# timdestan/go-raytracer

Measured on AMD Instinct MI355X. Metric: Mrays/s (primary+shadow+reflect) at 4K depth=6; 1/2/4/8-GPU scaling, higher is better.
Workload: dtype f64; 1 GPU; c3: cylinder + cube + sphere (cone substitute) over a reflective plane, 4 lights, 3840x2160, depth 6; width=3840, height=2160, depth=6, lights=4, objects=4, parallelism=rows1-interleaved, frames_in_flight=2, schedule=auto, kernel=specialised, accel=bvh+cull

## Files before the change

### go-raytracer_amd/csrc/rt_kernel.hip

```cpp
#pragma clang fp contract(off)

#include <hip/hip_runtime.h>

#include <dlfcn.h>
#include <errno.h>
#include <fcntl.h>
#include <hip/hiprtc.h>
#include <sys/syscall.h>
#include <sys/wait.h>
#include <unistd.h>

#include <algorithm>
#include <atomic>
#include <chrono>
#include <condition_variable>
#include <cstdlib>
#include <functional>
#include <thread>
#include <cmath>
#include <array>
#include <cstdio>
#include <utility>
#include <cstring>
#include <limits>
// ... 1962 lines not shown
  const std::array<int, 5> key = {y0, trow0, stride, tiles_x, tiles_y};
  auto it = c->orders.find(key);
  if (it != c->orders.end()) {
    *out = it->second;
    return RT_OK;
  }
  const DevScene& s = c->sc;
  const int ftx = (s.width + TILE - 1) / TILE, fty = (s.height + TILE - 1) / TILE;
  const int n = tiles_x * tiles_y;
  std::vector<uint32_t> cost(n), ord(n);
  for (int v = 0; v < n; v++) {
    const int tr = v / tiles_x, tc = v % tiles_x;
    int fr = stride > 0 ? trow0 + tr * stride : (y0 + tr * TILE + TILE / 2) / TILE;
    fr = std::min(fr, fty - 1);
    cost[v] = tc < ftx ? c->tile_cost[(size_t)fr * ftx + tc] : 0u;
    ord[v] = (uint32_t)v;
  }
  std::stable_sort(ord.begin(), ord.end(), [&](uint32_t a, uint32_t b) { return cost[a] > cost[b]; });
  static const int topd = rt_getenv("RT_ORDER_TOP") ? std::max(1, atoi(rt_getenv("RT_ORDER_TOP"))) : 6;
  static const int taild = rt_getenv("RT_ORDER_TAIL") ? std::max(0, atoi(rt_getenv("RT_ORDER_TAIL"))) : 0;
  {
    const int top = n / topd;
    const int tail = taild > 0 ? std::min(n - top, n / taild) : 0;
    std::vector<char> cls(n, 1);
    for (int i = 0; i < top; i++) cls[ord[i]] = 0;
    for (int i = n - tail; i < n; i++) cls[ord[i]] = 2;
    int k = top;
    for (int v = 0; v < n; v++)
      if (cls[v] == 1) ord[k++] = (uint32_t)v;
    for (int v = 0; v < n; v++)
      if (cls[v] == 2) ord[k++] = (uint32_t)v;
  }
  unsigned int* d = nullptr;
  HIP_TRY(hipMalloc((void**)&d, (size_t)n * sizeof(unsigned int)));
  if (hipMemcpy(d, ord.data(), (size_t)n * sizeof(unsigned int), hipMemcpyHostToDevice) != hipSuccess) {
    (void)hipFree(d);
    return fail(RT_E_DEVICE, "tile order upload failed");
  }
  c->orders[key] = d;
  *out = d;
  return RT_OK;
}

static int launch(rt_context* c, int y0, int y1, int trow0, int stride, int ntrows, void* d_rgba, void* stream,
                  bool est) {
  const DevScene& s = c->sc;
  DeviceGuard guard(c->device);
  hipStream_t st = (hipStream_t)stream;
  if (c->spec_pending && !est) (void)spec_prepare(c);
  const bool lds = scene_in_lds(s);
  const int vm_off = lds ? s.blob_bytes : 0;
  const int stack_off = vm_off + ((lds && s.num_programs) ? WG * MAT * (int)sizeof(double) : 0);
  const int cnt_off = stack_off + (s.use_bvh ? WAVES_PER_WG * BVH_STACK * 12 : 0);
  const int qmask_off = cnt_off + CNT_BYTES;
  const int jump_off = qmask_off + 16;
  const int board_off = jump_off + 20 * 4 * (int)sizeof(uint64_t);
  const uint64_t launch_pixels = (uint64_t)s.width * (uint64_t)(stride > 0 ? ntrows * TILE : y1 - y0);
  const int sch =
      est ? (int)SCH_SERIAL : pick_schedule(c->sched, s, launch_pixels, c->cus, c->inflight, c->spec_fn != nullptr);
  const int share_m = (c->spec_fn && !est) ? pick_share(c->share_mode, s, launch_pixels, c->cus, c->inflight) : 0;
  hipFunction_t spec = nullptr;
  if (!est) {
    int rc = spec_for(c, sch, share_m, &spec);
    if (rc != RT_OK) return rc;
  }
  static const bool spec_extra = rt_getenv("RT_SPEC_EXTRA_FLAGS") != nullptr;
  const bool use_stream = !lds && !s.use_bvh && !s.has_csg && (spec_extra || !(spec && !(c->accel & RT_ACCEL_CULL)));
  const bool quads = sch == SCH_QUADS || (sch == SCH_PAIRS && !spec);
  const void* kfn = k_kernels[kernel_index(lds, s.use_bvh, s.has_csg, quads, s.ext_code)];
  const bool share = spec && share_m == RT_SHARE_GROUP;
  const int stream_off = board_off + (share ? BOARD_BYTES : 0);
  const int frames_off = stream_off + (use_stream ? WAVES_PER_WG * SCH * (GEO * (int)sizeof(double) + (int)sizeof(int)) : 0);
  int shmem = frames_off;
  auto occupancy = [&](int bytes) {
    int n = 0;
    if (spec) {
      if (hipModuleOccupancyMaxActiveBlocksPerMultiprocessor(&n, spec, WG, bytes) != hipSuccess) n = 0;
    } else if (hipOccupancyMaxActiveBlocksPerMultiprocessor(&n, kfn, WG, bytes) != hipSuccess) {
      n = 0;
    }
    return n;
  };
  const void* plan_fn = spec ? (const void*)spec : kfn;
  const int frames = std::max(1, s.depth - 1);
  LaunchPlan& pl = c->plan;
  const bool plan_hit = pl.fn == plan_fn && pl.shmem_fixed == shmem && pl.frames == frames;
  int per_cu = plan_hit ? pl.per_cu : occupancy(shmem);
  if (per_cu <= 0) per_cu = 1;
  const int level_bytes = WAVES_PER_WG * CORE * 64 * (int)sizeof(double);
  int lds_levels = plan_hit ? pl.lds_levels : 0;
  if (!plan_hit && c->lds_per_cu > 0 && c->lds_per_block > 0) {
    const int avail = std::min(c->lds_per_block, c->lds_per_cu / std::min(per_cu, 8)) - shmem;
    lds_levels = std::max(0, std::min(frames, avail / level_bytes));
    if (const char* e = rt_getenv("RT_LDS_LEVELS")) lds_levels = std::max(0, std::min(lds_levels, atoi(e)));
    while (lds_levels > 0 && occupancy(shmem + lds_levels * level_bytes) < per_cu) lds_levels--;
  }
  if (!plan_hit) pl = LaunchPlan{plan_fn, shmem, frames, per_cu, lds_levels};
  shmem += lds_levels * level_bytes;
  static const bool dbg = rt_getenv("RT_DEBUG_LAUNCH") != nullptr;
  if (dbg)
    fprintf(stderr, "[launch] blocks/CU %d, LDS/block %d B (fixed %d, frame cores %d levels), frames %d\n", per_cu, shmem,
            frames_off, lds_levels, frames);
  const int grid = c->cus * std::min(per_cu, 8);
  c->last_waves = grid * WAVES_PER_WG;
  c->launches++;
  if (grid * WAVES_PER_WG > c->stack_waves) return fail(RT_E_INVALID, "frame stack smaller than the grid");
  if (spec && share_m == RT_SHARE_DEVICE) {
    const size_t need = (size_t)c->stack_waves * 64 * frames;
    if (need != c->gslots || frames != c->gframes) {
      (void)hipFree(c->gboard);
      c->gboard = nullptr;
      c->gslots = 0;
      if (hipExtMallocWithFlags((void**)&c->gboard, need * GS_REC * sizeof(uint64_t), hipDeviceMallocUncached) !=
          hipSuccess)
        return fail(RT_E_NOMEM, "device-wide work-sharing slots");
      if (!c->gring && hipExtMallocWithFlags((void**)&c->gring, (size_t)GS_RING * sizeof(uint64_t),
                                             hipDeviceMallocUncached) != hipSuccess)
        return fail(RT_E_NOMEM, "device-wide work-sharing ring");
// ... 384 lines not shown
```

### go-raytracer_amd/csrc/rt_render.h

```cpp
#pragma once
#pragma clang fp contract(off)

#ifndef __HIPCC_RTC__
#include <hip/hip_runtime.h>
#endif

#include "rt_abi.h"
#include "rt_device.h"

#ifndef RT_CULL
#define RT_CULL 1
#endif
#ifndef RT_SHARE
#define RT_SHARE 0
#endif
#ifndef RT_PAIRS
#define RT_PAIRS 0
#endif
#ifndef RT_FAR_SHIFT
#define RT_FAR_SHIFT 1
#endif
#ifndef RT_GS_POLL
#define RT_GS_POLL 3
#endif
// ... 58 lines not shown
#else
#define SHDIAG(k) (void)0
#endif
enum { S_IDLE = 0, S_TRACE = 1, S_SHADE = 2, S_DONE = 3 };
enum { LDS_MAX_BYTES = 40 * 1024 };
enum { JUMP_ENTRIES = 20 * 4 };

__device__ __forceinline__ int est_x(int pts, unsigned int k) { return pts == 1 ? TILE / 2 : 2 + 4 * (int)(k & 1u); }
__device__ __forceinline__ int est_y(int pts, unsigned int k) { return pts == 1 ? TILE / 2 : 2 + 4 * (int)((k >> 1) & 1u); }

struct Params {
  int lds_frames_off;
  int lds_levels;
  int stream_off;
  int qmask_off;
  int jump_off;
  int off_geo, off_shade, off_mats, off_lights, off_kind, off_objmat, off_pref, off_csg, off_code, off_consts,
      off_entry, blob_bytes;
  int lds_vm_off;
  double* vm_global;
  const uint64_t* jump;
  unsigned int* queue;
  unsigned int* queue_next;
  unsigned long long* stats;
  unsigned long long* stats_part;
  unsigned long long* wdiag;
  double* stack;
  uint32_t* out;
  int width, height, depth, nobj, nlights, y0, y1, tiles_x;
  int trow0, trow_stride;
  unsigned int total_slots;
  int frames;
  const float* bvh_nodes;
  const double* bvh_geo;
  const int* planes;
  int nplanes, bvh_stack_off;
  double bvh_lo[3], bvh_hi[3];
  const int* runs;
  int nruns;
  const double* arec;
  const double* urec;
  int cnt_off;
  int kind_mask;
  int board_off;
  uint64_t* gboard;
  uint64_t* gring;
  uint64_t* gctl;
  int gset;
  unsigned long long gslots;
  const unsigned int* order;
  unsigned int* est_out;
  int est_pts;
};
enum { CNT_TRACED = 0, CNT_SHADED = 1, CNT_SURFERR = 2, NUNIT = 3, CNT_KIND_OFF = 128,
       CNT_BYTES = CNT_KIND_OFF + RT_NUM_KINDS * WG * 8 };
enum { PREF = 8 };
enum { BN = 16, BVH_STACK = 64 };

struct Ray {
  d3 o, d;
};

template <typename MP>
__device__ __forceinline__ d3 to_obj_o(MP m, d3 o) {
  return mk(m[0] * o.x + m[1] * o.y + m[2] * o.z + m[3], m[4] * o.x + m[5] * o.y + m[6] * o.z + m[7],
            m[8] * o.x + m[9] * o.y + m[10] * o.z + m[11]);
}
template <typename MP>
__device__ __forceinline__ d3 to_obj_d(MP m, d3 d) {
  return mk(m[0] * d.x + m[1] * d.y + m[2] * d.z, m[4] * d.x + m[5] * d.y + m[6] * d.z,
            m[8] * d.x + m[9] * d.y + m[10] * d.z);
}
template <typename MP>
__device__ __forceinline__ Ray to_obj(MP m, const Ray& r) {
  Ray l;
  l.o = to_obj_o(m, r.o);
  l.d = to_obj_d(m, r.d);
  return l;
}
__device__ __forceinline__ bool ax_mag(double x, bool zero_ok) {
  const uint32_t e = ((uint32_t)__double2hiint(x) >> 20) & 0x7ffu;
  return e - 123u < 1800u || (zero_ok && x == 0.0);
}
__device__ __forceinline__ bool axis_o_ok(d3 o) { return ax_mag(o.x, true) && ax_mag(o.y, true) && ax_mag(o.z, true); }
__device__ __forceinline__ bool axis_d_ok(d3 d) { return ax_mag(d.x, false) && ax_mag(d.y, false) && ax_mag(d.z, false); }
__device__ __forceinline__ d3 axis_o(const double* a, d3 o) {
  return mk(a[0] * o.x + a[1], a[2] * o.y + a[3], a[4] * o.z + a[5]);
}
__device__ __forceinline__ d3 axis_d(const double* a, d3 d) { return mk(a[0] * d.x, a[2] * d.y, a[4] * d.z); }

typedef const __attribute__((address_space(4))) double* cdptr;
typedef const __attribute__((address_space(4))) float* cfptr;
typedef const __attribute__((address_space(4))) int* ciptr;
typedef __attribute__((address_space(3))) double* ldptr;
typedef __attribute__((address_space(1))) double* gdptr;
__device__ __forceinline__ const float* as_f(const double* p) { return reinterpret_cast<const float*>(p); }
__device__ __forceinline__ cfptr as_f(cdptr p) { return (cfptr)p; }
__device__ __forceinline__ const int* as_i(const double* p) { return reinterpret_cast<const int*>(p); }
__device__ __forceinline__ ciptr as_i(cdptr p) { return (ciptr)p; }
template <int N>
struct RecN {
  double m[N];
};
typedef RecN<12> Rec12;
typedef RecN<6> Rec6;
typedef RecN<3> Rec3;
enum { AXIS_REC = 8, UNI_REC = 4 };
template <int N, typename PT>
__device__ __forceinline__ RecN<N> ld_rec(PT p) {
// ... 1080 lines not shown
          }
          if (op == VM_EXT_REAL) {
            SETF((double)I_(a));
            break;
          }
        }
        return true;
    }
  }
#undef F_
#undef I_
#undef SETF
  return true;
}

__device__ __forceinline__ d3 combine(bool tmode, d3 lw, d3 col, double refl, double kr, d3 R, d3 Tr) {
  if (!tmode) return clamp(mul(add(lw, scale(R, refl)), col));
  return clamp(mul(add(lw, add(scale(R, kr), scale(Tr, 1.0 - kr))), col));
}

struct View {
  const int* entry;
  const uint32_t* code;
  const uint64_t* consts;
  const double* geo;
  const double* shade;
  const double* mats;
  const double* lights;
  const int* kind;
  const int* objmat;
  const uint32_t* pref;
  const int* csg;
};

enum { MIN_WAVES = RT_CULL ? 3 : 5 };
template <bool LDS, bool BVH, bool CSG, bool QUADS, bool EXT = true>
__global__ __launch_bounds__(WG, MIN_WAVES) void rt_render_kernel(const char* __restrict__ blob, Params P) {
  extern __shared__ __attribute__((aligned(16))) char smem[];
#ifdef RT_COST_MAP
  constexpr bool QD = false;
  constexpr bool PR = false;
#else
  constexpr bool QD = QUADS;
  constexpr bool PR = !QUADS && RT_PAIRS && RT_SHARE != 1;
#endif
  constexpr unsigned int QCHUNK = QD ? 16u : PR ? 32u : (unsigned int)QCHUNK_PIXEL;
  const char* base;
  uint64_t* jrows = reinterpret_cast<uint64_t*>(smem + P.jump_off);
  if constexpr (!QD)
    for (int i = threadIdx.x; i < 20 * 4; i += WG) jrows[i] = P.jump[(i >> 2) * 16 + (i & 3)];
  unsigned int* qdrained = reinterpret_cast<unsigned int*>(smem + P.qmask_off);
  if (threadIdx.x == 0) *qdrained = 0u;
  if (threadIdx.x < NUNIT * WAVES_PER_WG) reinterpret_cast<unsigned long long*>(smem + P.cnt_off)[threadIdx.x] = 0ull;
  Board* Bd = reinterpret_cast<Board*>(smem + P.board_off);
  if constexpr (RT_SHARE == 1) {
    if (threadIdx.x == 0) {
      Bd->post = 0ull;
      Bd->done = 0ull;
      Bd->nidle = 0;
      Bd->nactive = WAVES_PER_WG;
    }
    if (threadIdx.x < WAVES_PER_WG) Bd->wfree[threadIdx.x] = (1u << SLOTS_PER_WAVE) - 1u;
  }
  if (blockIdx.x == 0 && threadIdx.x < QHEADS) atomicExch(P.queue_next + threadIdx.x * QSTRIDE, 0u);
  const int gshard = (int)(blockIdx.x % (unsigned)GS_SH);
  uint64_t* const g_ring = P.gring + (size_t)gshard * GS_RSH;
  uint64_t* const g_head = P.gctl + GS_SHARD * gshard + GS_HEAD;
  uint64_t* const g_tail = P.gctl + GS_SHARD * gshard + GS_TAIL;
  uint64_t* const g_set = P.gctl + GS_SET + GS_SETSZ * P.gset;
  unsigned int* g_nidle = reinterpret_cast<unsigned int*>(g_set + GS_NIDLE + 512 * gshard);
  unsigned int* g_active = reinterpret_cast<unsigned int*>(g_set + GS_ACTIVE);
  unsigned int* g_helpers = reinterpret_cast<unsigned int*>(g_set + GS_HELPERS);
  auto nidle_add = [&](int delta) {
    if ((int)(threadIdx.x & 63) < GS_SH)
      atomicAdd(reinterpret_cast<unsigned int*>(g_set + GS_NIDLE + 512 * (threadIdx.x & 63)), (unsigned int)delta);
  };
  if constexpr (RT_SHARE == 2) {
    if (blockIdx.x == 0 && threadIdx.x < 2 + GS_SH)
      atomicExch(reinterpret_cast<unsigned int*>(P.gctl + GS_SET + GS_SETSZ * (1 - P.gset) + 512 * threadIdx.x), 0u);
    if ((threadIdx.x & 63) == 0) atomicAdd(g_active, 1u);
  }
  int gs_nid = 0;
  uint64_t gs_h = 0, gs_t = 0;
  bool gs_helper = false;
  if constexpr (LDS) {
    const int n16 = P.blob_bytes / 16;
    for (int i = threadIdx.x; i < n16; i += WG)
      reinterpret_cast<uint4*>(smem)[i] = reinterpret_cast<const uint4*>(blob)[i];
    base = smem;
  } else {
    base = blob;
  }
  __syncthreads();
  View S;
  S.geo = reinterpret_cast<const double*>(base + P.off_geo);
  S.shade = reinterpret_cast<const double*>(base + P.off_shade);
  S.mats = reinterpret_cast<const double*>(base + P.off_mats);
  const double* G = reinterpret_cast<const double*>(base + P.off_lights);
  S.lights = G + GLOB;
  S.kind = reinterpret_cast<const int*>(base + P.off_kind);
  S.objmat = reinterpret_cast<const int*>(base + P.off_objmat);
  S.pref = reinterpret_cast<const uint32_t*>(base + P.off_pref);
  S.csg = reinterpret_cast<const int*>(base + P.off_csg);
  S.code = reinterpret_cast<const uint32_t*>(base + P.off_code);
  S.entry = reinterpret_cast<const int*>(base + P.off_entry);
  S.consts = reinterpret_cast<const uint64_t*>(base + P.off_consts);
// ... 80 lines not shown
        pre[q] = idx < n16 ? src[(size_t)c0 * (GEO * sizeof(double) / 16) + idx] : make_uint4(0, 0, 0, 0);
      }
      pk = lane_ < min(SCH, P.nobj - c0) ? S.kind[c0 + lane_] : 0;
    };
    auto store = [&]() {
#pragma unroll
      for (int q = 0; q < PER; q++) dst[lane_ + q * 64] = pre[q];
      if (lane_ < SCH) skind[lane_] = pk;
      __builtin_amdgcn_fence(__ATOMIC_SEQ_CST, "wavefront");
    };
    if (P.nobj <= 0) return;
    fetch(0);
    store();
    for (int c0 = 0; c0 < P.nobj; c0 += SCH) {
      const int n = min(SCH, P.nobj - c0);
      const bool more = c0 + SCH < P.nobj;
      if (more) fetch(c0 + SCH);
      for (int j = 0; j < n; j++)
        if (!body(c0 + j, skind[j], sbuf + (size_t)j * GEO)) return;
      __builtin_amdgcn_fence(__ATOMIC_SEQ_CST, "wavefront");
      if (more) store();
    }
  };
  const d3 eye = mk(0.0, 0.0, -1.0);

  int state = S_IDLE;
  bool need_gen = false;
  int px = 0, py = 0, sample = 0, sp = 0;
  unsigned int pout = 0;
  uint32_t held_px = ~0u, held_val = 0u;
  auto flush_pixels = [&]() {
    if (held_px != ~0u) P.out[held_px] = held_val;
    held_px = ~0u;
  };
  constexpr bool WAVE_SGPR = BVH || CSG;
  const int wave = WAVE_SGPR ? __builtin_amdgcn_readfirstlane((int)(threadIdx.x >> 6)) : (int)(threadIdx.x >> 6);
  int my_idle = 0, spins = 0;
  bool my_active = true;
  bool sh_live = false;
  int hit_i = 0, hit_f = 0;
  double hit_t = 0.0;
  Pcg rng{0, 0};
  d3 sum = mk(0, 0, 0);
  d3 sum2 = mk(0, 0, 0);
  Ray ray;
  ray.o = mk(0, 0, 0);
  ray.d = mk(0, 0, 1);

  unsigned int pool_next = 0, pool_end = 0;
  int qhead = 0;
  bool exhausted = false;
  unsigned long long* cnt = reinterpret_cast<unsigned long long*>(smem + P.cnt_off);
  unsigned long long* kcnt = reinterpret_cast<unsigned long long*>(smem + P.cnt_off + CNT_KIND_OFF);
  for (int k = 0; k < RT_NUM_KINDS; k++) kcnt[k * WG + threadIdx.x] = 0;
  constexpr bool CNT_REMAT = BVH || CSG;
  auto opaque_s = [](uint32_t b) {
    b = (uint32_t)__builtin_amdgcn_readfirstlane((int)b);
    asm volatile("" : "+s"(b));
    return b;
  };
  auto cnt_kind = [&](int k, uint64_t v) {
    if constexpr (CNT_REMAT) {
      uint32_t l;
      asm volatile("v_mbcnt_lo_u32_b32 %0, -1, 0\n\tv_mbcnt_hi_u32_b32 %0, -1, %0" : "=v"(l));
      const uint32_t a = opaque_s((uint32_t)P.cnt_off + (uint32_t)(CNT_KIND_OFF + (k * WG + wave * 64) * 8)) + l * 8u;
      atomicAdd(reinterpret_cast<unsigned long long*>(smem + a), (unsigned long long)v);
    } else {
      atomicAdd(&kcnt[k * WG + threadIdx.x], (unsigned long long)v);
    }
  };
  auto cnt_unit = [&](int k, bool b) {
    const unsigned int n = (unsigned int)__popcll(wave_ballot(b));
    if (lane == 0 && n) {
      if constexpr (CNT_REMAT)
        atomicAdd(reinterpret_cast<unsigned long long*>(
                      smem + opaque_s((uint32_t)P.cnt_off + (uint32_t)((k * WAVES_PER_WG + wave) * 8))),
                  (unsigned long long)n);
      else
        atomicAdd(&cnt[k * WAVES_PER_WG + wave], (unsigned long long)n);
    }
  };
  WaveStack bst;
  bst.mask = reinterpret_cast<uint64_t*>(smem + P.bvh_stack_off) + (threadIdx.x >> 6) * BVH_STACK;
  bst.ref = reinterpret_cast<int*>(smem + P.bvh_stack_off + WAVES_PER_WG * BVH_STACK * 8) + (threadIdx.x >> 6) * BVH_STACK;
#ifdef RT_PHASE_TIMING
  uint64_t ph_acc[N_PHASE] = {0, 0, 0, 0, 0, 0, 0, 0, 0, 0};
  uint64_t bd_tnodes = 0, bd_snodes = 0, bd_tleaf = 0, bd_sleaf = 0, bd_trays = 0, bd_srays = 0;
  uint64_t pd_tr = 0, pd_trl = 0, pd_sh = 0, pd_shl = 0, pd_gen = 0, pd_genl = 0;
  uint64_t ld_done = 0, ld_rounds = 0;
#ifdef RT_COST_MAP
  uint32_t lane_cost = 0;
#endif
#endif

  const double W1 = (double)(P.width - 1), H1 = (double)(P.height - 1);

  auto gen_ray = [&]() {
    double dx = pcg_float64(rng) - 0.5;
    double dy = pcg_float64(rng) - 0.5;
    const double vw = G[9], vh = G[10];
    double u = ((double)px + dx) / W1 * vw - vw / 2.0;
    double v = ((double)py + dy) / H1 * vh - vh / 2.0;
    ray.o = mk(u, -v, 0.0);
    ray.d = norm(sub(ray.o, eye));
  };

  auto sample_rng = [&](int x, int y, int k) {
// ... 906 lines not shown
        double u, v;
        bool bad = false;
        long long face = (k == RT_PLANE) ? 0 : sf;
        if (k == RT_SPHERE) {
          bad = __builtin_fabs(p.y) > 1;
          v = (p.y + 1.0) / 2.0;
          u = go_acos(p.z / __builtin_sqrt(1.0 - p.y * p.y)) / 6.283185307179586;
        } else if ((k == RT_CYLINDER || k == RT_CONE) && sf == 0) {
          u = (go_atan2(p.x, p.z) + 3.141592653589793) / 6.283185307179586;
          v = p.y;
        } else {
          u = p.x;
          v = p.z;
        }
        double r[10];
        bad = run_vm<EXT>(S.code, S.consts, S.entry[-mat - 1], face, u, v, r) || bad;
        if (bad)
          for (int k = 0; k < 10; k++) r[k] = 0.0;
        vmrec[0] = r[0];
        vmrec[1] = r[1];
        vmrec[2] = r[2];
        vmrec[3] = r[3];
        const double fz = r[4];
        if (fz >= 0) {
          const double cf = go_cos(fz), sf = go_sin(fz);
          vmrec[4] = fz * cf * cf;
          vmrec[5] = fz * sf * sf;
          vmrec[6] = 1.0;
        } else {
          vmrec[4] = vmrec[5] = vmrec[6] = 0.0;
        }
        vmrec[7] = r[5];
        vmrec[8] = r[6];
        vmrec[9] = r[7];
        vmrec[10] = r[8];
        vmrec[11] = r[9];
        vmrec[12] = 1.0 / vmrec[8];
        const double r0 = (1.0 - vmrec[8]) / (1.0 + vmrec[8]);
        vmrec[13] = r0 * r0;
        surf_bad = bad;
      }
    }
    cnt_unit(CNT_SURFERR, surf_bad);

    PH_MARK(4);
    const double* M = (!spec_feat(SF_VM) || mat >= 0) ? S.mats + (size_t)mat * MAT : vmrec;
    d3 L = mk(0, 0, 0);
    if (hit) L = scale(mk(G[0], G[1], G[2]), M[9]);
    const double rlen = len(ray.d);
    const float rlen_rcpf = __builtin_amdgcn_rcpf((float)rlen);
    const d3 sorig = add(pw, scale(nw, 1e-4));
#define SH_PLANE_CULL(i, d, tmax) may_hit_plane(sof, d, tmax, SHP(i))
    uint32_t sc0 = 0, sc1 = 0, sc2 = 0, sc3 = 0;
    auto light_dir = [&](auto lt, d3& ldir, double& dist) {
      if (spec_feat(SF_LDIR) && (int)lt[9] == RT_LIGHT_DIRECTIONAL) {
        ldir = mk(lt[6], lt[7], lt[8]);
        dist = __builtin_inf();
      } else {
        d3 lth = sub(mk(lt[0], lt[1], lt[2]), pw);
        ldir = norm_len(lth, dist);
      }
    };
#ifdef RT_SPEC_NLIGHTS
    d3 ldir_a[RT_SPEC_NLIGHTS];
    double dist_a[RT_SPEC_NLIGHTS];
#pragma unroll
    for (int li = 0; li < RT_SPEC_NLIGHTS; li++) light_dir(LTP(li), ldir_a[li], dist_a[li]);
    PH_MARK(5);
#if !RT_CULL && !defined(RT_SPEC_NOBJ) && RT_SPEC_NLIGHTS <= 4
#define RT_JOINT_SWEEP 1
#else
#define RT_JOINT_SWEEP 0
#endif
#if RT_JOINT_SWEEP
    bool jopen[RT_SPEC_NLIGHTS];
    int jsend[RT_SPEC_NLIGHTS];
#pragma unroll
    for (int li = 0; li < RT_SPEC_NLIGHTS; li++) {
      jopen[li] = hit;
      jsend[li] = P.nobj;
    }
    if constexpr (STREAM) {
      const cdptr cgeo = (cdptr)S.geo;
      int lonm = 0;
      auto refresh = [&]() {
        int m = 0;
#pragma unroll
        for (int li = 0; li < RT_SPEC_NLIGHTS; li++) m |= wave_any(jopen[li]) ? (1 << li) : 0;
        lonm = __builtin_amdgcn_readfirstlane(m);
        return lonm != 0;
      };
      auto jsphere = [&](int i, const d3 lo, auto&& ldir) {
        const double c = dot(lo, lo) - 1.0;
#pragma unroll
        for (int li = 0; li < RT_SPEC_NLIGHTS; li++) {
          if (!((lonm >> li) & 1)) continue;
          const d3 ld = ldir(li);
          const double a = dot(ld, ld);
          const double hb = dot(lo, ld);
          const double disc = hb * hb - a * c;
          if (jopen[li] && !(disc < 0.0)) {
            const double t0 = (-hb - gsqrt(disc)) / a;
            if (t0 > 0.0 && t0 * rlen < dist_a[li] && i != hit_i) {
              jopen[li] = false;
              jsend[li] = i + 1;
            }
// ... 37 lines not shown
          };
          scan_uni<SHADOW_CHECK>((cdptr)P.urec, r0, rn, ubody, [&] { return !refresh(); });
        } else if (spec_kind(RT_SPHERE) && rk == RT_SPHERE && rax_k && sax) {
          scan_records<SHADOW_CHECK, 6, AXIS_REC>((cdptr)P.arec, r0, rn, [&](int i, const Rec6& R) {
            jsphere(i, axis_o(R.m, sorig), [&](int li) { return axis_d(R.m, ldir_a[li]); });
          }, [&] { return !refresh(); });
        } else if (spec_kind(RT_SPHERE) && rk == RT_SPHERE) {
          scan_records<SHADOW_CHECK>(cgeo, r0, rn, [&](int i, const Rec12& R) {
            jsphere(i, to_obj_o(R.m, sorig), [&](int li) { return to_obj_d(R.m, ldir_a[li]); });
          }, [&] { return !refresh(); });
        } else {
          for (int i = r0; i < r0 + rn; i++) {
#pragma unroll
            for (int li = 0; li < RT_SPEC_NLIGHTS; li++) {
              if (jopen[li] && i != hit_i) {
                Ray sr;
                sr.o = sorig;
                sr.d = ldir_a[li];
                double t;
                int f;
                if (object_hit(rk, S.geo + (size_t)i * GEO, sr, t, f) && t * rlen < dist_a[li]) {
                  jopen[li] = false;
                  jsend[li] = i + 1;
                }
              }
            }
          }
        }
      }
    }
#endif
#pragma unroll
    for (int li = 0; li < RT_SPEC_NLIGHTS; li++) {
      const auto lt = LTP(li);
      const int lkind = (int)lt[9];
      const d3 ldir = ldir_a[li];
      const double dist = dist_a[li];
#else
    for (int li = 0; li < P.nlights; li++) {
      const auto lt = LTP(li);
      const int lkind = (int)lt[9];
      d3 ldir;
      double dist;
      light_dir(lt, ldir, dist);
#endif
      bool open = hit;
      Ray sr;
      sr.o = sorig;
      sr.d = ldir;
      const F3 sof = f3(sorig), sdf = f3(ldir);
      const float sslack = ray_slack(sof);
      const float stmax = (float)dist * rlen_rcpf * 1.0001f + 1e-4f;
      int send = P.nobj;
      if constexpr (!BVH) {
#ifdef RT_SPEC_NOBJ
#pragma unroll
        for (int i = 0; i < RT_SPEC_NOBJ; i++) {
          if (!wave_any(open)) break;
          const int k = spec_kinds[i];
#else
        if constexpr (STREAM) {
#if defined(RT_SPEC_NLIGHTS) && RT_JOINT_SWEEP
          open = jopen[li];
          send = jsend[li];
#elif !RT_CULL
          const cdptr cgeo = (cdptr)S.geo;
          auto ssphere = [&](int i, const Ray& l) {
            const double a = dot(l.d, l.d);
            const double hb = dot(l.o, l.d);
            const double c = dot(l.o, l.o) - 1.0;
            const double disc = hb * hb - a * c;
            if (open && !(disc < 0.0)) {
              const double t0 = (-hb - gsqrt(disc)) / a;
              if (t0 > 0.0 && t0 * rlen < dist && i != hit_i) {
                open = false;
                send = i + 1;
              }
            }
          };
          const bool sax = wave_all(!hit || (axis_o_ok(sr.o) && axis_d_ok(sr.d)));
          for (int r = 0; r < P.nruns; r++) {
            if (!wave_any(open)) break;
            const int r0 = __builtin_amdgcn_readfirstlane(P.runs[4 * r]), rn = __builtin_amdgcn_readfirstlane(P.runs[4 * r + 1]),
                      rk = __builtin_amdgcn_readfirstlane(P.runs[4 * r + 2]), rax_k = __builtin_amdgcn_readfirstlane(P.runs[4 * r + 3]);
            if (spec_kind(RT_SPHERE) && rk == RT_SPHERE && rax_k == 2 && sax) {
              const double sc = ((cdptr)P.urec)[(size_t)r0 * UNI_REC + 3];
              const d3 so = mk(sc * sr.o.x, sc * sr.o.y, sc * sr.o.z);
              Ray l;
              l.d = mk(sc * sr.d.x, sc * sr.d.y, sc * sr.d.z);
              scan_records<SHADOW_CHECK, 3, UNI_REC>((cdptr)P.urec, r0, rn, [&](int i, const Rec3& R) {
                l.o = mk(so.x + R.m[0], so.y + R.m[1], so.z + R.m[2]);
                ssphere(i, l);
              }, [&] { return !wave_any(open); });
            } else if (spec_kind(RT_SPHERE) && rk == RT_SPHERE && rax_k && sax) {
              scan_records<SHADOW_CHECK, 6, AXIS_REC>((cdptr)P.arec, r0, rn, [&](int i, const Rec6& R) {
                Ray l;
                l.o = axis_o(R.m, sr.o);
                l.d = axis_d(R.m, sr.d);
                ssphere(i, l);
              }, [&] { return !wave_any(open); });
            } else if (spec_kind(RT_SPHERE) && rk == RT_SPHERE) {
              scan_records<SHADOW_CHECK>(cgeo, r0, rn, [&](int i, const Rec12& R) { ssphere(i, to_obj(R.m, sr)); },
                                            [&] { return !wave_any(open); });
            } else {
              for (int i = r0; i < r0 + rn; i++) {
                if (!wave_any(open)) break;
// ... 12 lines not shown
          stream_objects([&](int i, int k, const double* g) {
            if (!wave_any(open)) return false;
            bool test = CULL_AND(open, i != hit_i);
#if RT_CULL
            test = k != RT_PLANE ? may_hit_a(test, sof, sdf, stmax, g, sslack)
                                 : CULL_AND(test, may_hit_plane(sof, sdf, stmax, SHP(i)));
            if (!wave_any(test)) return true;
#endif
            EXDIAG(k, 1, test);
            if (test) {
              double t;
              int f;
              if (object_hit(k, g, sr, t, f) && t * rlen < dist) {
                open = false;
                send = i + 1;
              }
            }
            return true;
          });
#endif
        }
        for (int i = STREAM ? P.nobj : 0; i < P.nobj; i++) {
          if (!wave_any(open)) break;
          const int k = S.kind[i];
#endif
#ifdef RT_SPEC_NOBJ
          double gl[GEO];
#pragma unroll
          for (int q = 0; q < GEO; q++) gl[q] = sgeo[i * GEO + q];
          const double* g = gl;
#else
          const double* g = S.geo + (size_t)i * GEO;
#endif
          bool test = CULL_AND(open, i != hit_i);
#if RT_CULL
          test = k != RT_PLANE ? may_hit_a(test, sof, sdf, stmax, g, sslack)
                               : CULL_AND(test, SH_PLANE_CULL(i, sdf, stmax));
          if (!wave_any(test)) continue;
#endif
          EXDIAG(k, 1, test);
          if (test) {
            double t;
            int f;
            bool h;
            if constexpr (CSG)
              h = k == RT_CSG ? csg_hit<EXT>(CSG_ARGS, P.nobj, CSG_G(i, g), sr, t, f, rlen, dist, false)
                              : object_hit(k, g, sr, t, f);
            else
              h = object_hit(k, g, sr, t, f);
            if (h) {
              if (t * rlen < dist) {
                open = false;
                send = i + 1;
              }
            }
          }
        }
      } else {
        int occ = 0x7fffffff;
        auto shadow_exact = [&](int i, int k, const double* g, bool test) {
          EXDIAG(k, 1, test);
          if (test) {
            double t;
            int f;
            bool h;
            if constexpr (CSG)
              h = k == RT_CSG ? csg_hit<EXT>(CSG_ARGS, P.nobj, CSG_G(i, g), sr, t, f, rlen, dist, false)
                              : object_hit(k, g, sr, t, f);
            else
              h = object_hit(k, g, sr, t, f);
            if (h) {
              if (t * rlen < dist) occ = i;
            }
          }
        };
        auto shadow_obj = [&](int i, int k, const double* g, bool act) {
          bool test = CULL_AND(CULL_AND(act, i != hit_i), i < occ);
          test = k != RT_PLANE ? may_hit_a(test, sof, sdf, stmax, g, sslack)
                               : CULL_AND(test, may_hit_plane(sof, sdf, stmax, SHP(i)));
          if (!wave_any(test)) return;
          shadow_exact(i, k, g, test);
        };
        for (int p = 0; p < P.nplanes; p++) {
          const int i = P.planes[p];
          shadow_obj(i, S.kind[i], S.geo + (size_t)i * GEO, hit);
        }
        const F3 sidf = f3_rcp(sdf);
        F3 sbof = sof;
        float sbslack = sslack;
        double sbt0 = 0.0;
        bool sact = hit;
        far_shift(sact, sr, P.bvh_lo, P.bvh_hi, sbof, sbslack, sbt0);
        const float sbtmax = sbt0 == 0.0 ? stmax : (float)(dist / rlen - sbt0) * 1.0001f + 1e-4f;
#ifdef RT_PHASE_TIMING
        bd_srays++;
#endif
        int ssp = 0;
        int nr = 0;
        uint64_t nm = wave_ballot(sact);
        bool have = true;
        for (;;) {
          int r;
          uint64_t m;
          if (have) {
            r = nr;
            m = nm;
            have = false;
          } else {
            if (ssp == 0) break;
            ssp--;
            r = __builtin_amdgcn_readfirstlane(bst.ref[ssp]);
            m = ((uint64_t)__builtin_amdgcn_readfirstlane((int)(bst.mask[ssp] >> 32)) << 32) |
                (uint32_t)__builtin_amdgcn_readfirstlane((int)bst.mask[ssp]);
          }
          const bool act = sact && ((m >> lane) & 1);
#ifdef RT_PHASE_TIMING
          bd_snodes++;
#ifdef RT_COST_MAP
          if (hit) lane_cost++;
#endif
#endif
          if (r & 7) {
#ifdef RT_PHASE_TIMING
            bd_sleaf++;
#endif
            const int first = r >> 3, count = r & 7;
            for (int j = first; j < first + count; j++) {
              const LeafRec L = ld_leaf(P.bvh_geo, j);
              const bool test = may_hit_s(CULL_AND(CULL_AND(act, L.i != hit_i), L.i < occ), sbof, sdf, sbtmax, L.cx,
                                          L.cy, L.cz, L.cr, sbslack);
              if (!wave_any(test)) continue;
              shadow_exact(L.i, L.k, L.R.m, test);
            }
          } else {
            const cfptr nb = (cfptr)P.bvh_nodes + (size_t)(r >> 3) * BN;
            const ciptr ni = (ciptr)(nb + 12);
            float t0 = 0.0f, t1 = 0.0f;
            const bool a0 = may_hit_box_a(CULL_AND(act, ni[2] < occ), sbof, sidf, sbslack, sbtmax, nb, t0);
            const bool a1 = may_hit_box_a(CULL_AND(act, ni[3] < occ), sbof, sidf, sbslack, sbtmax, nb + 6, t1);
            const uint64_t m0 = wave_ballot(a0), m1 = wave_ballot(a1);
            const bool c1_first = ni[3] < ni[2];
            bvh_next(bst, ssp, lane, c1_first, ni[0], ni[1], m0, m1, nr, nm, have);
          }
        }
        open = hit && occ == 0x7fffffff;
        send = open ? P.nobj : occ + 1;
      }
      if (hit) {
        const uint4 pe = *reinterpret_cast<const uint4*>(S.pref + (size_t)send * PREF);
        const uint32_t pe4 = S.pref[(size_t)send * PREF + 4];
        const int hk = hit_i < send ? S.kind[hit_i] : -1;
        sc0 += pe.x - (hk == 0 ? 1u : 0u);
        sc1 += pe.y - (hk == 1 ? 1u : 0u);
        sc2 += pe.z - (hk == 2 ? 1u : 0u);
        sc3 += pe.w - (hk == 3 ? 1u : 0u);
        if (spec_kind(4) && (P.kind_mask & 16)) cnt_kind(4, pe4 - (hk == 4 ? 1u : 0u));
        if (spec_kind(5) && (P.kind_mask & 32)) cnt_kind(5, S.pref[(size_t)send * PREF + 5] - (hk == 5 ? 1u : 0u));
      }
      PH_MARK(6);
      if (hit && open) {
        d3 lcol = mk(lt[3], lt[4], lt[5]);
        if (spec_feat(SF_LSPOT) && lkind == RT_LIGHT_SPOT) {
          const double ca = dot(neg(ldir), mk(lt[6], lt[7], lt[8]));
          lcol = scale(lcol, ca >= lt[10] ? go_pow(ca, lt[11], (int)G[11]) : 0.0);
        }
        double ndl = go_max0(dot(nw, ldir));
        d3 diffuse = scale(lcol, ndl * M[9]);
        d3 H = norm(add(neg(ray.d), ldir));
        double spec = go_max0(dot(nw, H));
        d3 specular = scale(lcol, M[10] * go_pow(spec, M[11], (int)G[11]));
        L = add(add(L, diffuse), specular);
      }
      PH_MARK(7);
    }
    if (hit) {
      if (spec_kind(0) && (P.kind_mask & 1)) cnt_kind(0, sc0);
      if (spec_kind(1) && (P.kind_mask & 2)) cnt_kind(1, sc1);
      if (spec_kind(2) && (P.kind_mask & 4)) cnt_kind(2, sc2);
      if (spec_kind(3) && (P.kind_mask & 8)) cnt_kind(3, sc3);
    }

    bool have_res = false;
    d3 res = mk(0, 0, 0);
    if (hit) {
      d3 col = mk(M[0], M[1], M[2]);
      double refl = M[3], T = M[7];
      if (refl == 0 && T == 0) {
        res = clamp(mul(L, col));
        have_res = true;
      } else {
        bool hasR = refl > 0;
        Ray rr;
        rr.o = mk(0, 0, 0);
        rr.d = mk(0, 0, 1);
        if (hasR) {
          d3 rd = sub(ray.d, scale(nw, 2.0 * dot(ray.d, nw)));
          if (M[6] != 0.0) rd = add(rd, mk(M[4], M[5], 0.0));
          rr.o = sorig;
          rr.d = norm(rd);
        }
        bool tmode = T > 0;
        bool hasT = false;
        Ray trr;
        trr.o = mk(0, 0, 0);
        trr.d = mk(0, 0, 1);
        double kr = 0.0;
        d3 lw = L;
        if (tmode) {
          double ratio = M[12];
          d3 nn = nw;
          if (dot(ray.d, nn) > 0.0) {
            ratio = M[8];
            nn = scale(nn, -1.0);
          }
          double cosI = -dot(nn, ray.d);
          double sinT2 = ratio * ratio * (1.0 - cosI * cosI);
          if (!(sinT2 > 1.0)) {
            double cosT = gsqrt(1.0 - sinT2);
            d3 td = add(scale(ray.d, ratio), scale(nn, ratio * cosI - cosT));
            if (!iszero(td)) {
              hasT = true;
              trr.o = sub(pw, scale(nn, 1e-4));
              trr.d = td;
            }
          }
          double cosi = dot(ray.d, nw) / (rlen * len(nw));
          const double r0 = M[13];
          double cost = __builtin_fabs(cosi);
          kr = r0 + (1 - r0) * go_pow(1 - cost, 5);
          lw = scale(L, 1.0 - T);
        }
        const int d = P.depth - sp;
        if (d - 1 > 0 && (hasR || hasT)) {
          if (hasR && hasT) {
            const gdptr f = frame(sp);
            st3(f, FR_EXT, trr.o);
            st3(f, FR_EXT + 3, trr.d);
          }
          if (spec_feat(SF_VM) && mat < 0) {
            const gdptr f = frame(sp);
            st3(f, FR_COL, col);
            fr(f, FR_REFL) = refl;
          }
          long long packed = ((long long)(mat < 0 ? 0 : mat) << PK_MAT) | (mat < 0 ? FL_VMMAT : 0) |
                             (tmode ? FL_TMODE : 0) | (hasR ? FL_HASR : 0) | (hasT ? FL_HAST : 0);
          core_store(sp, packed, lw, kr);
          sp++;
          ray = hasR ? rr : trr;
          state = S_TRACE;
        } else {
          res = combine(tmode, lw, col, refl, kr, mk(0, 0, 0), mk(0, 0, 0));
          have_res = true;
        }
      }
    }
    PH_MARK(8);
    unwind(have_res, res, false, 0, mk(0, 0, 0), 0.0);
    PH_MARK(9);
  }
  flush_pixels();

  if (lane == 0) {
#ifdef RT_PHASE_TIMING
    for (int k = 0; k < N_PHASE; k++) atomicAdd(P.stats + ST_PHASE + k, (unsigned long long)ph_acc[k]);
    atomicAdd(P.stats + ST_BVHDIAG + 0, (unsigned long long)bd_tnodes);
    atomicAdd(P.stats + ST_BVHDIAG + 1, (unsigned long long)bd_snodes);
    atomicAdd(P.stats + ST_BVHDIAG + 2, (unsigned long long)bd_tleaf);
    atomicAdd(P.stats + ST_BVHDIAG + 3, (unsigned long long)bd_sleaf);
    atomicAdd(P.stats + ST_BVHDIAG + 4, (unsigned long long)bd_trays);
    atomicAdd(P.stats + ST_BVHDIAG + 5, (unsigned long long)bd_srays);
    atomicAdd(P.stats + ST_PASSDIAG + 0, (unsigned long long)pd_tr);
    atomicAdd(P.stats + ST_PASSDIAG + 1, (unsigned long long)pd_trl);
    atomicAdd(P.stats + ST_PASSDIAG + 2, (unsigned long long)pd_sh);
    atomicAdd(P.stats + ST_PASSDIAG + 3, (unsigned long long)pd_shl);
    atomicAdd(P.stats + ST_PASSDIAG + 4, (unsigned long long)pd_gen);
    atomicAdd(P.stats + ST_PASSDIAG + 5, (unsigned long long)pd_genl);
    atomicAdd(P.stats + ST_LANEDIAG + 0, (unsigned long long)ld_done);
    atomicAdd(P.stats + ST_LANEDIAG + 1, (unsigned long long)ld_rounds);
    const uint64_t t_end = stamp();
    const bool clock_ok = t_end >= life_t0;
    const uint64_t life = clock_ok ? t_end - life_t0 : 0;
    if (clock_ok) {
      atomicAdd(P.stats + ST_BVHDIAG + 6, (unsigned long long)life);
      atomicMax(P.stats + ST_BVHDIAG + 7, (unsigned long long)life);
    } else {
      atomicAdd(P.stats + ST_CLOCKSTEP, 1ull);
    }
    if (P.wdiag) {
      P.wdiag[(size_t)wslot * 4 + 0] = life;
      P.wdiag[(size_t)wslot * 4 + 1] = nchunk_taken;
      P.wdiag[(size_t)wslot * 4 + 2] = stamp() - last_grab;
    }
#endif
  }
  __syncthreads();
  unsigned long long* part = P.stats_part + (size_t)blockIdx.x * STATS_PART;
  if (!P.stats_part) {
  } else if (threadIdx.x < RT_NUM_KINDS) {
    unsigned long long sum = 0;
    for (int j = 0; j < WG; j++) sum += kcnt[threadIdx.x * WG + j];
    if (sum) part[ST_STESTS + threadIdx.x] += sum;
  } else if (threadIdx.x < RT_NUM_KINDS + NUNIT) {
    const int k = (int)threadIdx.x - RT_NUM_KINDS;
    unsigned long long sum = 0;
    for (int j = 0; j < WAVES_PER_WG; j++) sum += cnt[k * WAVES_PER_WG + j];
    const int slot = k == CNT_TRACED ? ST_TRACED : (k == CNT_SHADED ? ST_SHADED : ST_SURFERR);
    if (sum) part[slot] += sum;
    if (k == CNT_SHADED && sum) part[ST_SHADOW] += sum * (unsigned long long)P.nlights;
  }
}
```

Before: 75120 Mrays/s.

## Pack per-kind shadow-test tallies into byte fields and flush per wave

Replaces the per-thread 64-bit per-kind shadow-test counters with packed 8/16-bit fields held in registers, built from constexpr prefix tables indexed by the occluding object. The fields are periodically flushed with atomics into per-wave LDS slots, which shrinks the counter LDS region from WG to WAVES_PER_WG entries per kind. The goal is to cut per-pass counter work and LDS footprint, which may raise occupancy. The cost is extra register state, periodic LDS atomics, and host and device offset logic that must stay in sync.

```diff
diff --git a/go-raytracer_amd/csrc/rt_kernel.hip b/go-raytracer_amd/csrc/rt_kernel.hip
--- a/go-raytracer_amd/csrc/rt_kernel.hip
+++ b/go-raytracer_amd/csrc/rt_kernel.hip
@@ -2038,9 +2038,6 @@
   const int vm_off = lds ? s.blob_bytes : 0;
   const int stack_off = vm_off + ((lds && s.num_programs) ? WG * MAT * (int)sizeof(double) : 0);
   const int cnt_off = stack_off + (s.use_bvh ? WAVES_PER_WG * BVH_STACK * 12 : 0);
-  const int qmask_off = cnt_off + CNT_BYTES;
-  const int jump_off = qmask_off + 16;
-  const int board_off = jump_off + 20 * 4 * (int)sizeof(uint64_t);
   const uint64_t launch_pixels = (uint64_t)s.width * (uint64_t)(stride > 0 ? ntrows * TILE : y1 - y0);
   const int sch =
       est ? (int)SCH_SERIAL : pick_schedule(c->sched, s, launch_pixels, c->cus, c->inflight, c->spec_fn != nullptr);
@@ -2050,6 +2047,10 @@
     int rc = spec_for(c, sch, share_m, &spec);
     if (rc != RT_OK) return rc;
   }
+  const bool sc_packed = spec && c->spec_key.nobj > 0 && c->spec_key.nlights > 0;
+  const int qmask_off = cnt_off + cnt_bytes(sc_packed);
+  const int jump_off = qmask_off + 16;
+  const int board_off = jump_off + 20 * 4 * (int)sizeof(uint64_t);
   static const bool spec_extra = rt_getenv("RT_SPEC_EXTRA_FLAGS") != nullptr;
   const bool use_stream = !lds && !s.use_bvh && !s.has_csg && (spec_extra || !(spec && !(c->accel & RT_ACCEL_CULL)));
   const bool quads = sch == SCH_QUADS || (sch == SCH_PAIRS && !spec);
diff --git a/go-raytracer_amd/csrc/rt_render.h b/go-raytracer_amd/csrc/rt_render.h
--- a/go-raytracer_amd/csrc/rt_render.h
+++ b/go-raytracer_amd/csrc/rt_render.h
@@ -134,9 +134,53 @@
   unsigned int* est_out;
   int est_pts;
 };
-enum { CNT_TRACED = 0, CNT_SHADED = 1, CNT_SURFERR = 2, NUNIT = 3, CNT_KIND_OFF = 128,
-       CNT_BYTES = CNT_KIND_OFF + RT_NUM_KINDS * WG * 8 };
+enum { CNT_TRACED = 0, CNT_SHADED = 1, CNT_SURFERR = 2, NUNIT = 3, CNT_KIND_OFF = 128 };
+__host__ __device__ constexpr int cnt_bytes(bool packed) {
+  return CNT_KIND_OFF + RT_NUM_KINDS * (packed ? WAVES_PER_WG : WG) * 8;
+}
 enum { PREF = 8 };
+
+#if defined(RT_SPEC_NOBJ) && defined(RT_SPEC_NLIGHTS)
+constexpr bool SC_BUILD = true;
+static_assert(RT_SPEC_NOBJ >= 1 && RT_SPEC_NOBJ <= 8 && RT_SPEC_NLIGHTS >= 1 && RT_SPEC_NLIGHTS <= 8,
+              "packed tallies: a pass's 8-bit fields hold at most lights * objects <= 64");
+#ifndef RT_SC_FLUSH
+#define RT_SC_FLUSH (65535 / (RT_SPEC_NLIGHTS * RT_SPEC_NOBJ))
+#endif
+enum { SC_FLUSH = RT_SC_FLUSH, SC_NOBJ = RT_SPEC_NOBJ };
+static_assert(SC_FLUSH >= 1 && SC_FLUSH * RT_SPEC_NLIGHTS * RT_SPEC_NOBJ <= 65535, "RT_SC_FLUSH overflows a 16-bit field");
+struct ScTab {
+  int field[RT_NUM_KINDS];
+  int nfields;
+  uint32_t pk[2][RT_SPEC_NOBJ + 1];
+  uint32_t hit_fields;
+};
+constexpr ScTab sc_make() {
+  ScTab t{};
+  for (int k = 0; k < RT_NUM_KINDS; k++) {
+    t.field[k] = t.nfields;
+    t.nfields += (SPEC_KMASK >> k) & 1;
+  }
+  for (int s = 0; s < RT_SPEC_NOBJ; s++) {
+    const int f = t.field[spec_kinds[s]];
+    for (int w = 0; w < 2; w++) t.pk[w][s + 1] = t.pk[w][s] + ((f >> 2) == w ? 1u << (8 * (f & 3)) : 0u);
+    t.hit_fields |= (uint32_t)f << (4 * s);
+  }
+  return t;
+}
+constexpr ScTab SC = sc_make();
+static_assert((SPEC_KMASK >> RT_NUM_KINDS) == 0 && SC.nfields >= 1 && SC.nfields <= 8, "kinds");
+enum { SC_WORDS = SC.nfields > 4 ? 2 : 1 };
+#else
+constexpr bool SC_BUILD = false;
+enum { SC_FLUSH = 1, SC_WORDS = 1, SC_NOBJ = 0 };
+struct ScTab {
+  int field[RT_NUM_KINDS];
+  uint32_t pk[2][1];
+  uint32_t hit_fields;
+};
+constexpr ScTab SC{};
+#endif
 enum { BN = 16, BVH_STACK = 64 };
 
 struct Ray {
@@ -1323,6 +1367,10 @@
   unsigned int* qdrained = reinterpret_cast<unsigned int*>(smem + P.qmask_off);
   if (threadIdx.x == 0) *qdrained = 0u;
   if (threadIdx.x < NUNIT * WAVES_PER_WG) reinterpret_cast<unsigned long long*>(smem + P.cnt_off)[threadIdx.x] = 0ull;
+  constexpr bool SCP = SC_BUILD && !BVH && !CSG;
+  if constexpr (SCP)
+    if (threadIdx.x < RT_NUM_KINDS * WAVES_PER_WG)
+      reinterpret_cast<unsigned long long*>(smem + P.cnt_off + CNT_KIND_OFF)[threadIdx.x] = 0ull;
   Board* Bd = reinterpret_cast<Board*>(smem + P.board_off);
   if constexpr (RT_SHARE == 1) {
     if (threadIdx.x == 0) {
@@ -1509,7 +1557,22 @@
   bool exhausted = false;
   unsigned long long* cnt = reinterpret_cast<unsigned long long*>(smem + P.cnt_off);
   unsigned long long* kcnt = reinterpret_cast<unsigned long long*>(smem + P.cnt_off + CNT_KIND_OFF);
-  for (int k = 0; k < RT_NUM_KINDS; k++) kcnt[k * WG + threadIdx.x] = 0;
+  if constexpr (!SCP)
+    for (int k = 0; k < RT_NUM_KINDS; k++) kcnt[k * WG + threadIdx.x] = 0;
+  uint32_t sc_acc[2][2] = {{0u, 0u}, {0u, 0u}};
+  int sc_passes = 0;
+  auto sc_flush = [&]() {
+#pragma unroll
+    for (int k = 0; k < RT_NUM_KINDS; k++) {
+      if (!spec_kind(k)) continue;
+      const int f = SC.field[k];
+      const uint32_t v = (sc_acc[f >> 2][(f >> 1) & 1] >> (16 * (f & 1))) & 0xffffu;
+      atomicAdd(&kcnt[k * WAVES_PER_WG + wave], (unsigned long long)v);
+    }
+#pragma unroll
+    for (int w = 0; w < SC_WORDS; w++) sc_acc[w][0] = sc_acc[w][1] = 0u;
+    sc_passes = 0;
+  };
   constexpr bool CNT_REMAT = BVH || CSG;
   auto opaque_s = [](uint32_t b) {
     b = (uint32_t)__builtin_amdgcn_readfirstlane((int)b);
@@ -2522,6 +2585,15 @@
     const d3 sorig = add(pw, scale(nw, 1e-4));
 #define SH_PLANE_CULL(i, d, tmax) may_hit_plane(sof, d, tmax, SHP(i))
     uint32_t sc0 = 0, sc1 = 0, sc2 = 0, sc3 = 0;
+    uint32_t sc_hb[2] = {0u, 0u}, sc_full[2] = {0u, 0u}, sc_sum[2] = {0u, 0u};
+    if constexpr (SCP) {
+      const uint32_t hf = (SC.hit_fields >> (4 * (hit_i & 7))) & 7u;
+#pragma unroll
+      for (int w = 0; w < SC_WORDS; w++) {
+        sc_hb[w] = SC_WORDS == 1 ? 1u << (8 * hf) : ((hf >> 2) == (uint32_t)w ? 1u << (8 * (hf & 3u)) : 0u);
+        sc_full[w] = hit ? SC.pk[w][SC_NOBJ] - sc_hb[w] : 0u;
+      }
+    }
     auto light_dir = [&](auto lt, d3& ldir, double& dist) {
       if (spec_feat(SF_LDIR) && (int)lt[9] == RT_LIGHT_DIRECTIONAL) {
         ldir = mk(lt[6], lt[7], lt[8]);
@@ -2665,6 +2737,7 @@
       const float sslack = ray_slack(sof);
       const float stmax = (float)dist * rlen_rcpf * 1.0001f + 1e-4f;
       int send = P.nobj;
+      uint32_t spk[2] = {sc_full[0], sc_full[1]};
       if constexpr (!BVH) {
 #ifdef RT_SPEC_NOBJ
 #pragma unroll
@@ -2783,6 +2856,10 @@
               if (t * rlen < dist) {
                 open = false;
                 send = i + 1;
+                if constexpr (SCP) {
+#pragma unroll
+                  for (int w = 0; w < SC_WORDS; w++) spk[w] = SC.pk[w][i + 1] - (hit_i <= i ? sc_hb[w] : 0u);
+                }
               }
             }
           }
@@ -2877,7 +2954,10 @@
         open = hit && occ == 0x7fffffff;
         send = open ? P.nobj : occ + 1;
       }
-      if (hit) {
+      if constexpr (SCP) {
+#pragma unroll
+        for (int w = 0; w < SC_WORDS; w++) sc_sum[w] += spk[w];
+      } else if (hit) {
         const uint4 pe = *reinterpret_cast<const uint4*>(S.pref + (size_t)send * PREF);
         const uint32_t pe4 = S.pref[(size_t)send * PREF + 4];
         const int hk = hit_i < send ? S.kind[hit_i] : -1;
@@ -2904,7 +2984,14 @@
       }
       PH_MARK(7);
     }
-    if (hit) {
+    if constexpr (SCP) {
+#pragma unroll
+      for (int w = 0; w < SC_WORDS; w++) {
+        sc_acc[w][0] += __builtin_amdgcn_perm(0u, sc_sum[w], 0x0c010c00u);
+        sc_acc[w][1] += __builtin_amdgcn_perm(0u, sc_sum[w], 0x0c030c02u);
+      }
+      if (++sc_passes >= SC_FLUSH) sc_flush();
+    } else if (hit) {
       if (spec_kind(0) && (P.kind_mask & 1)) cnt_kind(0, sc0);
       if (spec_kind(1) && (P.kind_mask & 2)) cnt_kind(1, sc1);
       if (spec_kind(2) && (P.kind_mask & 4)) cnt_kind(2, sc2);
@@ -2990,6 +3077,7 @@
     PH_MARK(9);
   }
   flush_pixels();
+  if constexpr (SCP) sc_flush();
 
   if (lane == 0) {
 #ifdef RT_PHASE_TIMING
@@ -3029,7 +3117,8 @@
   if (!P.stats_part) {
   } else if (threadIdx.x < RT_NUM_KINDS) {
     unsigned long long sum = 0;
-    for (int j = 0; j < WG; j++) sum += kcnt[threadIdx.x * WG + j];
+    constexpr int per_kind = SCP ? WAVES_PER_WG : WG;
+    for (int j = 0; j < per_kind; j++) sum += kcnt[threadIdx.x * per_kind + j];
     if (sum) part[ST_STESTS + threadIdx.x] += sum;
   } else if (threadIdx.x < RT_NUM_KINDS + NUNIT) {
     const int k = (int)threadIdx.x - RT_NUM_KINDS;
```

After: 77170 Mrays/s, median of 6. 1.03x the previous value.
